# ojcharles/WeightedLD

Measured on AMD Instinct MI355X. Metric: LD site-pairs/sec at N=2000 seq × L=20000 var sites; 1/2/4/8 GPU; %HBM roofline, higher is better.
Workload: dtype fp6 (e2m3) weights x fp4 (e2m1) codes on block-scaled MFMA, screen (f32 sums, exact on the rounded weights; rigorous f32 r2 bound over every pair); candidate tiles (0 of 49144): f32 sums in lib.rs's order on f32 MFMA, f32 epilogue

## Files before the change

weightedld_amd/csrc/pair_mfma.hip:

```cpp
#include <algorithm>
#include <type_traits>
#include <vector>

#include "fp6_pack.hpp"
#include "pair_common.hpp"


namespace wld {

typedef int v4i __attribute__((ext_vector_type(4)));
typedef int v16i __attribute__((ext_vector_type(16)));

bool mfma_supported() { return true; }

namespace {
constexpr int kGroup = 8;
constexpr int kStageCodes = 4096;
constexpr int kDigStage = 128;
constexpr int kMaxPlanes = 4;
constexpr uint32_t kPlanes012 = 0 | (1 << 2) | (2 << 4);
constexpr int kDigGroup = 1024;
template <int NPL>
struct GroupShape {
    static constexpr int kStages = NPL == 1 ? 4 : kGroup;
// ... 821 lines not shown
    }
}
template <bool kShared>
__device__ __forceinline__ void f6c_rebuild(v4f (&acc)[4][2][2], const float2 *sA, const float2 *sB, uint32_t wq,
                                            uint32_t lane, float W6, float wv) {
    float col[4], mb[4];
#pragma unroll
    for (int n = 0; n < 4; ++n) {
        const float2 b = sB[(lane & 15) + 16 * n];
        col[n] = f6c_col_term(b.x, b.y);
        mb[n] = b.y;
    }
#pragma unroll
    for (int e = 0; e < 4; ++e) {
        const float2 a = sA[16 * wq + 4 * (lane >> 4) + e];
        f6c_rebuild_row<kShared>(acc, e, f6c_row_term(W6, a.x), 2.0f * a.y, col, mb, wv);
    }
}
struct F6Site {
    const F6RowRec *row;
    const F6ColRec *col;
    const F6MinRec *rmin, *cmin;
};
template <bool kShared, bool kCounts>
__device__ __forceinline__ void f6c_rebuild_rec(v4f (&acc)[4][2][2], const F6Site &st, uint32_t wq, uint32_t lane,
                                                float wv) {
    float col[4], mb[4];
#pragma unroll
    for (int n = 0; n < 4; ++n) {
        const F6tCol &b = st.col[(lane & 15) + 16 * n].b;
        col[n] = kCounts ? b.col * wv : b.col;
        mb[n] = kCounts ? b.mb * wv : b.mb;
    }
#pragma unroll
    for (int e = 0; e < 4; ++e) {
        const F6tRow &a = st.row[16 * wq + 4 * (lane >> 4) + e].a;
        f6c_rebuild_row<kShared>(acc, e, kCounts ? a.row * wv : a.row, kCounts ? a.ma2 * wv : a.ma2, col, mb, wv);
    }
}
template <bool kShared, bool kCounts>
__device__ __forceinline__ bool f6t_any_doubt(const v4f (&acc)[4][2][2], const F6Epi &ep, const F6Site &st, float wv) {
    F6tCol cb[4];
#pragma unroll
    for (int n = 0; n < 4; ++n) cb[n] = st.col[(ep.lane & 15) + 16 * n].b;
    auto terms = [&](const F6tRow &ra, int n, int e, float &mlo) {
        float p = acc[n][0][1][e], s = acc[n][1][0][e], t = acc[n][1][1][e];
        if constexpr (kCounts)
            p *= 0.5f;
        else if constexpr (kShared)
            p *= 0.5f * wv, s *= wv, t *= wv;
        return r2_screen_terms_f6t(p, s, t, ra, cb[n], ep.thr_c, ep.E, mlo);
    };
    if (ep.okA == ~0ull && ep.okB == ~0ull && ep.ta != ep.tb) {
        int worst = -1;
        float mlo_all = INFINITY;
#pragma unroll
        for (int e = 0; e < 4; ++e) {
            const F6tRow ra = st.row[16 * ep.wq + 4 * (ep.lane >> 4) + e].a;
#pragma unroll
            for (int n = 0; n < 4; ++n) {
                float mlo;
                worst = max(worst, __float_as_int(terms(ra, n, e, mlo)));
                mlo_all = fminf(mlo_all, mlo);
            }
        }
        return worst > 0 || !(mlo_all >= ep.mloc);
    }
    bool doubt = false;
#pragma unroll
    for (int e = 0; e < 4; ++e) {
        const F6tRow ra = st.row[16 * ep.wq + 4 * (ep.lane >> 4) + e].a;
#pragma unroll
        for (int n = 0; n < 4; ++n) {
            float mlo;
            const float t1 = terms(ra, n, e, mlo);
            if (ep.valid_pair(4 * n + e) && (t1 > 0.0f || !(mlo >= ep.mloc))) doubt = true;
        }
    }
    return doubt;
}
struct F6qCol {
    float mb, col, cW;
};
template <bool kShared, bool kCounts>
__device__ __forceinline__ bool f6t_quick_skip(const v4f (&acc)[4][2][2], const F6Epi &ep, const F6Site &st,
                                               const F6qCol (&cb)[4], const F6qColMin &cm, float wv) {
    const uint32_t grp = 4 * ep.wq + (ep.lane >> 4);
    F6qAcc q;
#pragma unroll
    for (int e = 0; e < 4; ++e) {
        const F6tRow &ra = st.row[4 * grp + e].a;
        const float ma2 = ra.ma2, row = ra.row;
#pragma unroll
        for (int n = 0; n < 4; ++n) {
            float p = acc[n][0][1][e], s = acc[n][1][0][e], t = acc[n][1][1][e];
            if constexpr (kShared && !kCounts) p *= 0.5f * wv, s *= wv, t *= wv;
            f6q_pair1<kCounts>(p, s, t, ma2, row, cb[n].mb, cb[n].col, cb[n].cW, q);
            __builtin_amdgcn_sched_barrier(0);
        }
    }
    f6q_pmax<kCounts>(q);
    const F6MinRec r = st.rmin[grp];
    float mlo;
    const float t1 = f6q_lane_terms(q, F6qRowMin{r.x, r.y, r.z}, cm, ep.thr_c, ep.E, mlo);
    return __ballot(!f6q_skip(t1, mlo, ep.mloc)) == 0;
}
template <bool kShared, bool kQuick, bool kCounts>
__device__ __forceinline__ bool f6t_wave_doubt(v4f (&acc)[2][4][2][2], const F6Epi &ep0, const F6Epi &ep1,
                                               const F6Site &st, float wv, uint32_t *full) {
    if constexpr (kQuick) {
        bool full0 = true, full1 = true;
        if (ep0.ta != ep0.tb) {
            F6qCol cb[4];
#pragma unroll
            for (int n = 0; n < 4; ++n) {
                const F6ColRec &b = st.col[(ep0.lane & 15) + 16 * n];
                cb[n] = F6qCol{b.b.mb, b.b.col, b.cW};
            }
            const F6MinRec c = st.cmin[ep0.lane & 15];
            const F6qColMin cm{c.x, c.y, c.z};
            full0 = !f6t_quick_skip<kShared, kCounts>(acc[0], ep0, st, cb, cm, wv);
            full1 = !f6t_quick_skip<kShared, kCounts>(acc[1], ep1, st, cb, cm, wv);
            if ((full0 || full1) && ep0.lane == 0) atomicAdd(full, (uint32_t)full0 + (uint32_t)full1);
        }
        uint32_t lane = ep0.lane;
        asm volatile("" : "+v"(lane), "+s"(wv)::"memory");
#pragma unroll
        for (int j = 0; j < 2; ++j)
#pragma unroll
            for (int n = 0; n < 4; ++n) asm volatile("" : "+v"(acc[j][n][1][1]));
        F6Epi e0 = ep0, e1 = ep1;
        e0.lane = e1.lane = lane;
        return (full0 && f6t_any_doubt<kShared, kCounts>(acc[0], e0, st, wv)) ||
               (full1 && f6t_any_doubt<kShared, kCounts>(acc[1], e1, st, wv));
    }
    return f6t_any_doubt<kShared, kCounts>(acc[0], ep0, st, wv) || f6t_any_doubt<kShared, kCounts>(acc[1], ep1, st, wv);
}
}

template <int kFmt>
__global__ __launch_bounds__(256, 4) void pair_fp6_screen_kernel(const uint8_t *__restrict__ a6,
                                                                  const uint8_t *__restrict__ b6,
                                                                  const float2 *__restrict__ marg, float W6,
                                                                  const uint64_t *__restrict__ ok_bits,
                                                                  const uint32_t *__restrict__ tiles, uint32_t n_tiles,
                                                                  uint32_t NK, uint32_t L, uint32_t n_chunk_rows,
                                                                  float thr, OrderArgs o, ScreenArgs sc, float wv) {
    using F = F6Fmt<kFmt>;
    constexpr int kF6AStage = F::kAStage, kF6ABytes = F::kABytes, kF6Stage = F::kStage;
    __shared__ __attribute__((aligned(16))) uint8_t smem[2 * kF6Stage];
    __shared__ float2 sMarg[2 * kTile];
    __shared__ unsigned long long sMask;
    __shared__ uint32_t sBail;
    if (!sc.probe && blockIdx.x == 0 && threadIdx.x == 0) *sc.cand_work = 0u;
    const uint32_t tid = threadIdx.x, lane = tid & 63, wave = __builtin_amdgcn_readfirstlane(tid >> 6);
    const uint32_t lds = lds_addr(smem), lane16 = lane * 16;
    const uint32_t ei = sc.probe ? blockIdx.x * sc.probe_stride + blockIdx.x % sc.probe_stride : blockIdx.x;
    const uint32_t tile = ei < n_tiles ? tiles[ei] : kNoTile;
    if (tile == kNoTile) return;
    const uint32_t ta = tile >> 16, tb = tile & 0xFFFFu;
    const uint8_t *sA = a6 + (size_t)ta * NK * kF6AStage, *sB = b6 + (size_t)tb * NK * kF6BStage;
    auto issue = [&](uint32_t kb, uint32_t buf) {
        const uint32_t gb = lds + buf * kF6Stage;
        const uint8_t *a = sA + (size_t)kb * kF6AStage, *b = sB + (size_t)kb * kF6BStage;
#pragma unroll
        for (uint32_t p = wave; p < kF6Stage / 1024; p += 4)
            glds16_s(p < kF6AStage / 1024 ? a + p * 1024 : b + (p - kF6AStage / 1024) * kF6BBytes, lane16, gb + p * 1024);
    };
    issue(0, 0);
    if (tid < 2 * kTile) sMarg[tid] = marg[(tid < kTile ? ta : tb) * kTile + (tid & (kTile - 1))];
    if (tid == 0) {
        uint32_t v = 0;
        if (sc.bail) {
            const unsigned cc = __hip_atomic_load(sc.cand_count, __ATOMIC_RELAXED, __HIP_MEMORY_SCOPE_AGENT);
            v = cc > sc.bail ? ((cc & kAbandonBit) ? 2u : 1u) : 0u;
        }
        sBail = v;
    }
    asm volatile("s_waitcnt lgkmcnt(0)" ::: "memory");
    const uint64_t okA = ok_bits[ta], okB = ok_bits[tb];
    v4f acc[4][2][2];
#pragma unroll
    for (int n = 0; n < 4; ++n)
#pragma unroll
        for (int x = 0; x < 2; ++x)
#pragma unroll
            for (int y = 0; y < 2; ++y) acc[n][x][y] = v4f{0.0f, 0.0f, 0.0f, 0.0f};
    uint32_t buf = 0;
    for (uint32_t kb = 0; kb < NK; ++kb) {
        asm volatile("s_waitcnt vmcnt(0)" ::: "memory");
        __builtin_amdgcn_s_barrier();
        asm volatile("" ::: "memory");
        if (kb == 0 && sBail) {
            if (tid == 0 && sBail == 1) {
                atomicOr(sc.cand_count, kAbandonBit);
                atomicOr(sc.cand_buckets, kAbandonBit);
            }
            asm volatile("s_waitcnt vmcnt(0)" ::: "memory");
            return;
        }
        if (kb + 1 < NK) issue(kb + 1, buf ^ 1);
        const uint8_t *g = smem + buf * kF6Stage;
        v8i ai, am;
        f6_ld_rows<kFmt>(g + wave * kF6ABytes, lane, ai, am);
#pragma unroll
        for (int n = 0; n < 4; ++n)
            f6_block_mfma<F::kCbsz>(acc[n], ai, am, f6_ldb(g + kF6AStage + n * kF6BBytes, lane));
        asm volatile("s_waitcnt lgkmcnt(0)" ::: "memory");
        buf ^= 1;
    }
    f6c_rebuild<F::kShared>(acc, sMarg, sMarg + kTile, wave, lane, W6, wv);
    const F6Epi ep{ta, tb, wave, lane, okA, okB, 2.0f * sc.Rf, thr * (1.0f - 0x1p-7f), sc.E, sc.mloc};
    const bool cand = ep.any(acc);
    if (sc.probe) {
        const bool any = __syncthreads_or(cand);
        if (tid == 0) {
            if (any) atomicAdd(sc.probe, 1u);
            atomicAdd(sc.probe + 1, 1u);
        }
        return;
    }
    if (tid == 0) sMask = 0ull;
    if (__syncthreads_or(cand)) {
        const unsigned mk = ep.blocks(acc);
        if (mk) atomicOr(&sMask, (unsigned long long)mk);
        __syncthreads();
        screen_verdict((uint32_t)sMask, ta, tb, tid, n_chunk_rows, o, sc);
    } else {
        screen_verdict(0u, ta, tb, tid, n_chunk_rows, o, sc);
    }
}

constexpr uint32_t kF6Single = 0x8000u;

#ifdef WLD_EXP_CLOCK
constexpr uint32_t kF6ClockSlots = 8192;
__device__ unsigned long long gF6Clock[2 * kF6ClockSlots];
extern "C" int wld_debug_f6_clock(unsigned long long *out) {
    return (int)hipMemcpyFromSymbol(out, HIP_SYMBOL(gF6Clock), sizeof(gF6Clock));
}
#endif
struct F6Recs {
    const F6ColRec *col;
    const F6RowRec *row;
    const F6MinRec *rmin, *cmin;
    float inv;
};
constexpr int kF6SiteCol = 0, kF6SiteRow = 2 * kTile * sizeof(F6ColRec), kF6SiteRmin = kF6SiteRow + kTile * sizeof(F6RowRec),
              kF6SiteCmin = kF6SiteRmin + kTile / 4 * sizeof(F6MinRec),
              kF6SiteBytes = kF6SiteCmin + 2 * 16 * sizeof(F6MinRec);
static_assert(sizeof(F6ColRec) == 32 && sizeof(F6RowRec) == 24 && sizeof(F6MinRec) == 16 && kF6SiteBytes == 6400 &&
                  kF6SiteRow % 16 == 0 && kF6SiteRmin % 16 == 0,
              "the entry's records are staged as 400 16-byte pieces");
__device__ __forceinline__ F6Site f6_site_of(const uint8_t *site, uint32_t half) {
    return F6Site{reinterpret_cast<const F6RowRec *>(site + kF6SiteRow),
                  reinterpret_cast<const F6ColRec *>(site + kF6SiteCol) + kTile * half,
                  reinterpret_cast<const F6MinRec *>(site + kF6SiteRmin),
                  reinterpret_cast<const F6MinRec *>(site + kF6SiteCmin) + 16 * half};
}
template <int kFmt, bool kThree = false, bool kQuick = false, bool kCounts = false>
__global__ __launch_bounds__(256, 3) void pair_fp6_screen2w_kernel(
    const uint8_t *__restrict__ a6, const uint8_t *__restrict__ b6, const float2 *__restrict__ marg, float W6,
    const uint64_t *__restrict__ ok_bits,
    const uint32_t *__restrict__ pairs, uint32_t n_pairs, uint32_t NK, uint32_t L, uint32_t n_chunk_rows, float thr,
    OrderArgs o, ScreenArgs sc, float wv, F6Recs rec) {
    using F = F6Fmt<kFmt>;
    constexpr int kF6AStage = F::kAStage, kF6ABytes = F::kABytes, kF6PStage = F::kPStage;
    static_assert(!kCounts || (kThree && F::kShared), "count units: the shared image's three-sum tests");
    __shared__ __attribute__((aligned(16))) uint8_t smem[2 * kF6PStage];
    __shared__ __attribute__((aligned(kThree ? 16 : 8))) uint8_t sSite[kThree ? kF6SiteBytes : 3 * kTile * sizeof(float2)];
    const float2 *const sMarg = reinterpret_cast<const float2 *>(sSite);
    __shared__ unsigned long long sMask[2];
    __shared__ uint32_t sBail, sCand[2];
    __shared__ uint32_t sDoubt[2];
    __shared__ uint32_t sQuickFull;
    static_assert(kThree || !kQuick, "the quick test stands in front of the three-sum test");
    if (!sc.probe && blockIdx.x == 0 && threadIdx.x == 0) *sc.cand_work = 0u;
    const uint32_t tid = threadIdx.x, lane = tid & 63, wave = __builtin_amdgcn_readfirstlane(tid >> 6);
    const uint32_t half = wave >> 1, rp = wave & 1, ltid = tid & 127;
    const uint32_t lds = lds_addr(smem), lane16 = lane * 16;
    const uint32_t ei = sc.probe ? blockIdx.x * sc.probe_stride + blockIdx.x % sc.probe_stride : blockIdx.x;
    const uint32_t entry = ei < n_pairs ? pairs[ei] : kNoTile;
    if (entry == kNoTile) return;
    constexpr int kAPieces = kFmt == kF6A6 ? 3 : kFmt == kF6A4 ? 2 : 1;
    static_assert(kF6AStage == kAPieces * 4096 && kF6BStage == 4096, "five (fp4 A: four, shared: three) pieces per wave and stage");
    struct Src {
        const uint8_t *pA, *pB0, *pB1;
    };
    auto src_of = [&](uint32_t e) {
        const uint32_t ta_ = e >> 16, tb0_ = e & 0x7FFFu;
        Src r;
        r.pA = a6 + (size_t)ta_ * NK * kF6AStage + wave * 1024;
        r.pB0 = b6 + (size_t)tb0_ * NK * kF6BStage + wave * 1024;
        r.pB1 = (e & kF6Single) ? r.pB0 : r.pB0 + (size_t)NK * kF6BStage;
        return r;
    };
    auto issue = [&](const Src &sr, uint32_t kb, uint32_t buf) {
        const uint32_t gb = lds + buf * kF6PStage + wave * 1024;
        const uint8_t *a = sr.pA + (size_t)kb * kF6AStage;
        const size_t bo = (size_t)kb * kF6BStage;
        glds16_s(a, lane16, gb);
        if (kAPieces > 1) glds16_s(a + 4096, lane16, gb + 4096);
        if (kAPieces > 2) glds16_s(a + 8192, lane16, gb + 8192);
        glds16_s(sr.pB0 + bo, lane16, gb + kF6AStage);
        glds16_s(sr.pB1 + bo, lane16, gb + kF6AStage + kF6BStage);
    };
    const Src cur = src_of(entry);
    issue(cur, 0, 0);
    uint32_t buf = 0;
    {
        const uint32_t ta = entry >> 16, tb0 = entry & 0x7FFFu;
        const bool single = (entry & kF6Single) != 0, idle = single && half;
        const uint32_t tb = tb0 + (idle ? 0u : half);
        if constexpr (kThree) {
            const uint32_t tb1 = tb0 + (single ? 0u : 1u);
            uint4 *const dst = reinterpret_cast<uint4 *>(sSite);
            dst[tid] = reinterpret_cast<const uint4 *>(rec.col + (tid < 128 ? tb0 : tb1) * kTile)[tid & 127];
            if (tid < 96)
                dst[kF6SiteRow / 16 + tid] = reinterpret_cast<const uint4 *>(rec.row + ta * kTile)[tid];
            else if (tid < 112)
                dst[kF6SiteRmin / 16 + (tid - 96)] = reinterpret_cast<const uint4 *>(rec.rmin + ta * (kTile / 4))[tid - 96];
            else if (tid < 144)
                dst[kF6SiteCmin / 16 + (tid - 112)] =
                    reinterpret_cast<const uint4 *>(rec.cmin + (tid < 128 ? tb0 : tb1) * 16)[tid & 15];
        } else if (tid < 3 * kTile) {
            const uint32_t t = tid < kTile ? ta : tb0 + ((tid >= 2 * kTile && !single) ? 1u : 0u);
            reinterpret_cast<float2 *>(sSite)[tid] = marg[t * kTile + (tid & (kTile - 1))];
        }
        if (tid == 0) {
            uint32_t v = 0;
            if (sc.bail) {
                const unsigned cc = __hip_atomic_load(sc.cand_count, __ATOMIC_RELAXED, __HIP_MEMORY_SCOPE_AGENT);
                v = cc > sc.bail ? ((cc & kAbandonBit) ? 2u : 1u) : 0u;
            }
            sBail = v;
        }
        if constexpr (kThree)
            if (tid < 2) sDoubt[tid] = 0u;
        if constexpr (kQuick)
            if (tid == 2) sQuickFull = 0u;
        asm volatile("s_waitcnt lgkmcnt(0)" ::: "memory");
        const uint64_t okA = ok_bits[ta], okB = ok_bits[tb];
        v4f acc[2][4][2][2];
        const uint32_t boff = kF6AStage + (idle ? 0u : half) * kF6BStage;
        const uint32_t aoff = 2 * rp * kF6ABytes;
        auto stage = [&](uint32_t kb, auto first) -> bool {
            constexpr bool kFirst = decltype(first)::value;
            asm volatile("s_waitcnt vmcnt(0)" ::: "memory");
            __builtin_amdgcn_s_barrier();
            asm volatile("" ::: "memory");
            if (kFirst) {
                if (sBail) {
                    if (tid == 0 && sBail == 1) {
                        atomicOr(sc.cand_count, kAbandonBit);
                        atomicOr(sc.cand_buckets, kAbandonBit);
                    }
                    asm volatile("s_waitcnt vmcnt(0)" ::: "memory");
                    return false;
                }
                if (tid < 2) sCand[tid] = 0u, sMask[tid] = 0ull;
            }
            if (kb + 1 < NK) issue(cur, kb + 1, buf ^ 1);
            const uint8_t *g = smem + buf * kF6PStage;
            v8i ai0, am0, ai1, am1;
            f6_ld_rows<kFmt>(g + aoff, lane, ai0, am0);
            f6_ld_rows<kFmt>(g + aoff + kF6ABytes, lane, ai1, am1);
            const v4f kZero = {0.0f, 0.0f, 0.0f, 0.0f};
            v8i bs[2] = {f6_ldb(g + boff, lane), f6_ldb(g + boff + kF6BBytes, lane)};
#pragma unroll
            for (int n = 0; n < 4; ++n) {
                v8i &b = bs[n & 1];
                constexpr int kMinor = 0x22222222;
                if constexpr (!kThree) acc[0][n][0][0] = f6_mfma<F::kCbsz>(ai0, b, kFirst ? kZero : acc[0][n][0][0]);
                acc[0][n][1][0] = f6_mfma<F::kCbsz>(am0, b, kFirst ? kZero : acc[0][n][1][0]);
                if constexpr (!kThree) acc[1][n][0][0] = f6_mfma<F::kCbsz>(ai1, b, kFirst ? kZero : acc[1][n][0][0]);
                acc[1][n][1][0] = f6_mfma<F::kCbsz>(am1, b, kFirst ? kZero : acc[1][n][1][0]);
                __builtin_amdgcn_sched_barrier(0);
                b = v8i{b[0] & kMinor, b[1] & kMinor, b[2] & kMinor, b[3] & kMinor, 0, 0, 0, 0};
                acc[0][n][0][1] = f6_mfma<F::kCbsz>(ai0, b, kFirst ? kZero : acc[0][n][0][1]);
                acc[0][n][1][1] = f6_mfma<F::kCbsz>(am0, b, kFirst ? kZero : acc[0][n][1][1]);
                acc[1][n][0][1] = f6_mfma<F::kCbsz>(ai1, b, kFirst ? kZero : acc[1][n][0][1]);
                acc[1][n][1][1] = f6_mfma<F::kCbsz>(am1, b, kFirst ? kZero : acc[1][n][1][1]);
                __builtin_amdgcn_sched_barrier(0);
                if (n + 2 < 4) b = f6_ldb(g + boff + (n + 2) * kF6BBytes, lane);
                __builtin_amdgcn_sched_barrier(0);
            }
            asm volatile("s_waitcnt lgkmcnt(0)" ::: "memory");
            buf ^= 1;
            return true;
        };
#ifdef WLD_EXP_CLOCK
        const unsigned long long ck0 = clock64(), rt0 = wall_clock64();
#endif
        if (!stage(0, std::true_type{})) return;
        for (uint32_t kb = 1; kb < NK; ++kb) stage(kb, std::false_type{});
#ifdef WLD_EXP_CLOCK
        if (tid == 0) {
            gF6Clock[2 * (blockIdx.x % kF6ClockSlots)] = clock64() - ck0;
            gF6Clock[2 * (blockIdx.x % kF6ClockSlots) + 1] = wall_clock64() - rt0;
        }
#endif
        const F6Epi ep0{ta, tb, 2 * rp, lane, okA, okB, 2.0f * sc.Rf, thr * (1.0f - 0x1p-7f), sc.E, sc.mloc};
        const F6Epi ep1{ta, tb, 2 * rp + 1, lane, okA, okB, 2.0f * sc.Rf, thr * (1.0f - 0x1p-7f), sc.E, sc.mloc};
        if constexpr (kThree) {
            const F6Site st = f6_site_of(sSite, half);
            F6Epi t0 = ep0, t1 = ep1;
            t0.E = t1.E = kCounts ? sc.E * rec.inv * rec.inv : sc.E;
            t0.mloc = t1.mloc = kCounts ? sc.mloc * rec.inv : sc.mloc;
            const bool doubt =
                !idle && f6t_wave_doubt<F::kShared, kQuick, kCounts>(acc, t0, t1, st, wv, &sQuickFull);
            if (doubt) sDoubt[half] = 1u;
            __syncthreads();
            if constexpr (kQuick) {
                unsigned *const cnt = sc.probe ? sc.probe + 3 : sc.rechecked ? sc.rechecked + 1 : nullptr;
                if (tid == 0 && cnt && sQuickFull) atomicAdd(cnt, sQuickFull);
            }
#ifdef WLD_EXP_ZERO_IMG
            const bool again = (sDoubt[0] | sDoubt[1]) == 0x5EEDu;
#else
            const bool again = (sDoubt[0] | sDoubt[1]) != 0;
#endif
            if (!again) {
                if (sc.probe) {
                    if (ltid == 0 && !idle) atomicAdd(sc.probe + 1, 1u);
                } else if (!idle) {
                    screen_verdict(0u, ta, tb, ltid, n_chunk_rows, o, sc);
                }
                return;
            }
            if (unsigned *const cnt = sc.probe ? sc.probe + 2 : sc.rechecked; tid == 0 && cnt) atomicAdd(cnt, 1u);
#pragma unroll
            for (int n = 0; n < 4; ++n) acc[0][n][0][0] = acc[1][n][0][0] = v4f{0.0f, 0.0f, 0.0f, 0.0f};
            issue(cur, 0, buf);
            for (uint32_t kb = 0; kb < NK; ++kb) {
                asm volatile("s_waitcnt vmcnt(0)" ::: "memory");
                __builtin_amdgcn_s_barrier();
                asm volatile("" ::: "memory");
                if (kb + 1 < NK) issue(cur, kb + 1, buf ^ 1);
                const uint8_t *g = smem + buf * kF6PStage;
                v8i ai0, ai1;
                if constexpr (F::kShared) {
                    v8i am0, am1;
                    f6_ld_rows<kFmt>(g + aoff, lane, ai0, am0);
                    f6_ld_rows<kFmt>(g + aoff + kF6ABytes, lane, ai1, am1);
                } else {
                    ai0 = f6_lda<kFmt>(g + aoff, lane);
                    ai1 = f6_lda<kFmt>(g + aoff + kF6ABytes, lane);
                }
#pragma unroll
                for (int n = 0; n < 4; ++n) {
                    const v8i b = f6_ldb(g + boff + n * kF6BBytes, lane);
                    acc[0][n][0][0] = f6_mfma<F::kCbsz>(ai0, b, acc[0][n][0][0]);
                    acc[1][n][0][0] = f6_mfma<F::kCbsz>(ai1, b, acc[1][n][0][0]);
                }
                asm volatile("s_waitcnt lgkmcnt(0)" ::: "memory");
                buf ^= 1;
            }
        }
        if (!idle) {
            if constexpr (kThree) {
                const F6Site st = f6_site_of(sSite, half);
                f6c_rebuild_rec<F::kShared, kCounts>(acc[0], st, 2 * rp, lane, wv);
                f6c_rebuild_rec<F::kShared, kCounts>(acc[1], st, 2 * rp + 1, lane, wv);
            } else {
                f6c_rebuild<F::kShared>(acc[0], sMarg, sMarg + kTile * (1 + half), 2 * rp, lane, W6, wv);
                f6c_rebuild<F::kShared>(acc[1], sMarg, sMarg + kTile * (1 + half), 2 * rp + 1, lane, W6, wv);
            }
        }
        const bool cand = !idle && (ep0.any(acc[0]) || ep1.any(acc[1]));
        if (cand) sCand[half] = 1u;
        __syncthreads();
#ifdef WLD_EXP_ZERO_IMG
        const bool mine = sCand[half] == 0x5EEDu;
#else
        const bool mine = sCand[half] != 0;
#endif
        if (sc.probe) {
            if (ltid == 0 && !idle) {
                if (mine) atomicAdd(sc.probe, 1u);
                atomicAdd(sc.probe + 1, 1u);
            }
            return;
        }
        if (mine && !idle) {
            const unsigned mk = ep0.blocks(acc[0]) | ep1.blocks(acc[1]);
            if (mk) atomicOr(&sMask[half], (unsigned long long)mk);
        }
        __syncthreads();
        if (!idle) screen_verdict(mine ? (uint32_t)sMask[half] : 0u, ta, tb, ltid, n_chunk_rows, o, sc);
    }
}

constexpr int kI8ABytes = 2048;
constexpr int kI8AStage = 4 * kI8ABytes;
constexpr int kI8BStage = 4 * 1024;
constexpr int kI8PStage = kI8AStage + 2 * kI8BStage;
size_t i8_a_bytes(size_t LP, size_t NP) { return LP / 64 * (NP / 64) * kI8AStage; }
size_t i8_b_bytes(size_t LP, size_t NP) { return LP / 64 * (NP / 64) * kI8BStage; }

__global__ __launch_bounds__(256) void i8img_kernel(const uint8_t *__restrict__ codes, const int8_t *__restrict__ digit,
                                                     uint32_t LP, uint32_t NP, uint8_t *__restrict__ a8,
                                                     uint8_t *__restrict__ b8) {
    const uint32_t NK = NP / 64;
    const size_t idx = (size_t)blockIdx.x * 256 + threadIdx.x;
    if (idx >= (size_t)LP / 16 * NK * 64) return;
    const uint32_t lane = idx & 63, blk = (idx >> 6) & 3;
    const size_t tk = idx >> 8, tile = tk / NK;
    const uint32_t kb = (uint32_t)(tk % NK);
    const uint32_t k0 = 64 * kb + 16 * (lane >> 4);
    const uint4 c4 = *reinterpret_cast<const uint4 *>(codes + (tile * 64 + blk * 16 + (lane & 15)) * (size_t)NP + k0);
    const uint4 d4 = *reinterpret_cast<const uint4 *>(digit + k0);
    const uint32_t c[4] = {c4.x, c4.y, c4.z, c4.w}, d[4] = {d4.x, d4.y, d4.z, d4.w};
    uint32_t ai[4], am[4], b[4];
#pragma unroll
    for (int q = 0; q < 4; ++q) {
        uint32_t vi = 0, vm = 0, vb = 0;
#pragma unroll
        for (int j = 0; j < 4; ++j) {
            const uint32_t cc = (c[q] >> (8 * j)) & 0xFFu, dd = (d[q] >> (8 * j)) & 0xFFu;
            vi |= ((cc & kCodeIn) ? dd : 0u) << (8 * j);
            vm |= ((cc & kCodeMaj) ? dd : 0u) << (8 * j);
            vb |= ((cc & kCodeIn) ? ((cc & kCodeMaj) ? 2u : 1u) : 0u) << (8 * j);
        }
        ai[q] = vi, am[q] = vm, b[q] = vb;
    }
    uint8_t *pa = a8 + tk * kI8AStage + blk * kI8ABytes;
    *reinterpret_cast<uint4 *>(pa + 16 * lane) = make_uint4(ai[0], ai[1], ai[2], ai[3]);
    *reinterpret_cast<uint4 *>(pa + 1024 + 16 * lane) = make_uint4(am[0], am[1], am[2], am[3]);
    *reinterpret_cast<uint4 *>(b8 + tk * kI8BStage + blk * 1024 + 16 * lane) = make_uint4(b[0], b[1], b[2], b[3]);
}

void launch_i8img(const uint8_t *codes, const int8_t *digit, size_t LP, size_t NP, uint8_t *a8, uint8_t *b8,
                  hipStream_t s) {
    const size_t n = LP / 16 * (NP / 64) * 64;
    hipLaunchKernelGGL(i8img_kernel, dim3((unsigned)((n + 255) / 256)), dim3(256), 0, s, codes, digit, (uint32_t)LP,
                       (uint32_t)NP, a8, b8);
}

__global__ __launch_bounds__(256, 3) void pair_i8_screen2w_kernel(
    const uint8_t *__restrict__ a8, const uint8_t *__restrict__ b8, const uint64_t *__restrict__ ok_bits,
    const uint32_t *__restrict__ pairs, uint32_t n_pairs, uint32_t NK, uint32_t L, uint32_t n_chunk_rows, float thr,
    OrderArgs o, ScreenArgs sc) {
    __shared__ __attribute__((aligned(16))) uint8_t smem[2 * kI8PStage];
    __shared__ unsigned long long sMask[2];
    __shared__ uint32_t sCand[2];
    if (blockIdx.x == 0 && threadIdx.x == 0) *sc.cand_work = 0u;
    const uint32_t tid = threadIdx.x, lane = tid & 63, wave = __builtin_amdgcn_readfirstlane(tid >> 6);
    const uint32_t half = wave >> 1, rp = wave & 1, ltid = tid & 127;
    const uint32_t lds = lds_addr(smem), lane16 = lane * 16;
    const uint32_t entry = blockIdx.x < n_pairs ? pairs[blockIdx.x] : kNoTile;
    if (entry == kNoTile) return;
    const uint32_t ta = entry >> 16, tb0 = entry & 0x7FFFu;
    const bool single = (entry & kF6Single) != 0, idle = single && half;
    const uint32_t tb = tb0 + (idle ? 0u : half);
    static_assert(kI8AStage == 2 * 4096 && kI8BStage == 4096, "four pieces per wave and stage");
    const uint8_t *pA = a8 + (size_t)ta * NK * kI8AStage + wave * 1024;
    const uint8_t *pB0 = b8 + (size_t)tb0 * NK * kI8BStage + wave * 1024;
    const uint8_t *pB1 = single ? pB0 : pB0 + (size_t)NK * kI8BStage;
    auto issue = [&](uint32_t kb, uint32_t buf) {
        const uint32_t gb = lds + buf * kI8PStage + wave * 1024;
        const uint8_t *a = pA + (size_t)kb * kI8AStage;
        const size_t bo = (size_t)kb * kI8BStage;
        glds16_s(a, lane16, gb);
// ... 171 lines not shown
    hipLaunchKernelGGL(frag_kernel, dim3((unsigned)((chunks + 255) / 256)), dim3(256), 0, s, codes, (uint32_t)LP,
                       (uint32_t)NP, frag);
}

int mfma_weight_stats(const int8_t *wplanes, size_t LP, size_t NP, hipStream_t s, MfmaWeightStats *out) {
    struct {
        unsigned mask, pad;
        unsigned long long resid[3];
        unsigned long long dsum[kMaxPlanes];
    } h{};
    if (hipMemcpyAsync(&h, wplanes + planemask_offset(LP, NP), sizeof(h), hipMemcpyDeviceToHost, s) != hipSuccess ||
        hipStreamSynchronize(s) != hipSuccess)
        return -1;
    out->plane_mask = h.mask & 15;
    out->nonneg = !(h.mask & 0x100);
    for (int t = 0; t < 3; ++t) out->resid[t] = h.resid[t];
    for (int p = 0; p < kMaxPlanes; ++p) out->dsum[p] = h.dsum[p];
    return 0;
}

namespace {
template <int MODE, int NPL, bool LOOP = false>
void launch_lds(const MfmaLaunch &m, const uint64_t *ok_bits, const uint32_t *tiles, uint32_t n_tiles,
                const unsigned *tile_count, uint32_t grid, uint32_t plane_idx, const OrderArgs &o, const DenseArgs &dn,
                const ScreenArgs &sc, hipStream_t s) {
    hipLaunchKernelGGL((pair_mfma_kernel<MODE, NPL, LOOP>), dim3(grid), dim3(64 * GroupShape<NPL>::kWaves), 0, s, m.frag, m.frag_b, m.wplanes,
                       ok_bits, tiles, n_tiles, tile_count, m.L, m.NP, m.n_chunk_rows, m.thr, m.shift, plane_idx, o,
                       dn, sc);
}

template <int MODE, bool LOOP = false>
void launch_lds_planes(uint32_t n_planes, const MfmaLaunch &m, const uint64_t *ok_bits, const uint32_t *tiles,
                       uint32_t n_tiles, const unsigned *tile_count, uint32_t grid, uint32_t plane_idx,
                       const OrderArgs &o, const DenseArgs &dn, const ScreenArgs &sc, hipStream_t s) {
    if (n_planes == 4)
        launch_lds<MODE, 4, LOOP>(m, ok_bits, tiles, n_tiles, tile_count, grid, plane_idx, o, dn, sc, s);
    else if (n_planes == 3)
        launch_lds<MODE, 3, LOOP>(m, ok_bits, tiles, n_tiles, tile_count, grid, plane_idx, o, dn, sc, s);
    else if (n_planes == 2 || LOOP)
        launch_lds<MODE, 2, LOOP>(m, ok_bits, tiles, n_tiles, tile_count, grid, plane_idx, o, dn, sc, s);
    else
        launch_lds<MODE, 1, false>(m, ok_bits, tiles, n_tiles, tile_count, grid, plane_idx, o, dn, sc, s);
}
void launch_candidates(const MfmaLaunch &m, uint32_t n, uint32_t idx, const uint64_t *ok_bits, const OrderArgs &o,
                       const DenseArgs &dn, const ScreenArgs &sc, hipStream_t s) {
    if (m.test_guard && sc.cand_buckets && m.cand_list && sc.cand_bits && sc.cand_cap) {
        const size_t cap = sc.cand_cap, last = 16 * (size_t)m.n_tiles / cap - 1;
        (void)hipMemsetD32Async(reinterpret_cast<hipDeviceptr_t>(m.cand_list + last * cap), 0, cap, s);
        (void)hipMemsetD32Async(reinterpret_cast<hipDeviceptr_t>(sc.cand_bits + last * cap), 0, cap, s);
        (void)hipMemsetD32Async(reinterpret_cast<hipDeviceptr_t>(sc.cand_buckets + last), (int)(cap + 1), 1, s);
        if (m.cand_count)
            (void)hipMemsetD32Async(reinterpret_cast<hipDeviceptr_t>(m.cand_count), (int)(16 * m.n_tiles + 2), 1, s);
    }
    if (m.ref_valu) {
        ValuLaunch v = *m.ref_valu;
        v.tiles = m.cand_list;
        v.n_tiles = m.n_tiles;
        v.tile_count = m.cand_count;
        v.tile_bits = sc.cand_bits;
        v.tile_work = sc.cand_work;
        v.tile_buckets = sc.cand_buckets;
        v.bucket_cap = sc.cand_cap;
        v.rb_items = sc.rb_items != 0;
        v.scan = sc.scan;
        launch_pair_valu(v, o, nullptr, s);
        return;
    }
    const uint32_t grid = std::min<uint32_t>(m.n_tiles, kCandidateGrid);
    launch_lds_planes<kModePrefilter, true>(n, m, ok_bits, m.cand_list, 0, m.cand_count, grid, idx, o, dn, sc, s);
}
}

namespace {
void fp6_screen_args(const MfmaLaunch &m, ScreenArgs &sc) {
    sc.R = fp6_screen_R(*m.fp6);
    sc.Rf = (float)sc.R;
    sc.f32 = 2;
    screen_consts(m.fp6->Tg, 2.0f * sc.Rf, sc.E, sc.mloc);
}
template <int kFmt>
void launch_fp6_screen_fmt(const MfmaLaunch &m, const uint64_t *ok_bits, const OrderArgs &o, const ScreenArgs &sc,
                           uint32_t stride, hipStream_t s) {
    const bool counts = kFmt == kF6Shared && m.fp6->counts;
    const F6Recs rec = fp6_recs_of(m.fp6->rec, m.LP, counts ? 1.0f / m.fp6->wv : 1.0f);
    auto pairs = [&](auto kernel) {
        hipLaunchKernelGGL(kernel, dim3((m.f6_n_pairs + stride - 1) / stride), dim3(256), 0, s, m.fp6->a6, m.fp6->b6,
                           reinterpret_cast<const float2 *>(m.fp6->marg), m.fp6->W6, ok_bits, m.f6_pairs, m.f6_n_pairs,
                           m.fp6->NK, m.L, m.n_chunk_rows, m.thr, o, sc, m.fp6->wv, rec);
    };
    if (m.f6_pairs && m.fp6_three && m.fp6_quick) {
        if constexpr (kFmt == kF6Shared) {
            if (counts) return pairs(pair_fp6_screen2w_kernel<kFmt, true, true, true>);
        }
        pairs(pair_fp6_screen2w_kernel<kFmt, true, true>);
    } else if (m.f6_pairs && m.fp6_three) {
        if constexpr (kFmt == kF6Shared) {
            if (counts) return pairs(pair_fp6_screen2w_kernel<kFmt, true, false, true>);
        }
        pairs(pair_fp6_screen2w_kernel<kFmt, true>);
    } else if (m.f6_pairs) {
        pairs(pair_fp6_screen2w_kernel<kFmt>);
    } else {
        hipLaunchKernelGGL(pair_fp6_screen_kernel<kFmt>, dim3((m.n_tiles + stride - 1) / stride), dim3(256), 0, s,
                           m.fp6->a6, m.fp6->b6, reinterpret_cast<const float2 *>(m.fp6->marg), m.fp6->W6, ok_bits,
                           m.tiles, m.n_tiles, m.fp6->NK, m.L, m.n_chunk_rows, m.thr,
                           o, sc, m.fp6->wv);
    }
}
void launch_fp6_screen(const MfmaLaunch &m, const uint64_t *ok_bits, const OrderArgs &o, const ScreenArgs &sc,
                       uint32_t stride, hipStream_t s) {
    if (m.fp6->shared)
        launch_fp6_screen_fmt<kF6Shared>(m, ok_bits, o, sc, stride, s);
    else if (m.fp6->a4)
        launch_fp6_screen_fmt<kF6A4>(m, ok_bits, o, sc, stride, s);
    else
        launch_fp6_screen_fmt<kF6A6>(m, ok_bits, o, sc, stride, s);
}
}

void launch_fp6_probe(const MfmaLaunch &m, unsigned *probe, uint32_t stride, hipStream_t s) {
    const uint64_t *ok_bits = reinterpret_cast<const uint64_t *>(m.wplanes + okbits_offset(m.NP));
    ScreenArgs sc{};
    sc.nonneg = m.nonneg;
    fp6_screen_args(m, sc);
    sc.probe = probe;
    sc.probe_stride = std::max<uint32_t>(stride, 1);
    (void)hipMemsetAsync(probe, 0, 4 * sizeof(unsigned), s);
    launch_fp6_screen(m, ok_bits, OrderArgs{}, sc, sc.probe_stride, s);
}

void launch_pair_mfma(const MfmaLaunch &m, const OrderArgs &o, const DenseArgs *dense, hipStream_t s,
                      hipEvent_t screen_done) {
    using screen_policy::Route;
    const DenseArgs dn = dense ? *dense : DenseArgs{nullptr, nullptr, nullptr, nullptr};
    const uint64_t *ok_bits = reinterpret_cast<const uint64_t *>(m.wplanes + okbits_offset(m.NP));
    ScreenArgs sc{0.0,         0.0f,         0.0f,      0.0f,        0, m.nonneg, m.cand_list, m.cand_count,
                  m.cand_list + 16 * (size_t)m.n_tiles, m.cand_work, m.cand_buckets, m.n_tiles, 0, ScanArgs{}};
    if (!m.frag) {
        const dim3 g(m.n_tiles), b(256);
        if (dense)
            hipLaunchKernelGGL((pair_mfma_rows_kernel<kModeDense>), g, b, 0, s, m.codes, m.wplanes, ok_bits, m.tiles,
                               m.L, m.NP, m.n_chunk_rows, m.thr, m.shift, o, dn, sc);
        else if (m.bound_test)
            hipLaunchKernelGGL((pair_mfma_rows_kernel<kModePrefilter>), g, b, 0, s, m.codes, m.wplanes, ok_bits,
                               m.tiles, m.L, m.NP, m.n_chunk_rows, m.thr, m.shift, o, dn, sc);
        else
            hipLaunchKernelGGL((pair_mfma_rows_kernel<kModeAll>), g, b, 0, s, m.codes, m.wplanes, ok_bits, m.tiles,
                               m.L, m.NP, m.n_chunk_rows, m.thr, m.shift, o, dn, sc);
        return;
    }
    unsigned mask = m.plane_mask & 15;
    if (!mask) mask = 15;
    uint32_t idx = 0, n = 0, top = 0;
    for (uint32_t p = 0; p < kMaxPlanes; ++p)
        if (mask >> p & 1) idx |= p << (2 * n++), top = p;
    if (n == 3 && idx != kPlanes012) n = 4;
    if (n == 4) idx = 0 | (1 << 2) | (2 << 4) | (3 << 6);
    if (dense) {
        launch_lds_planes<kModeDense>(n, m, ok_bits, m.tiles, m.n_tiles, nullptr, m.n_tiles, idx, o, dn, sc, s);
        return;
    }
    if (!m.bound_test) {
        launch_lds_planes<kModeAll>(n, m, ok_bits, m.tiles, m.n_tiles, nullptr, m.n_tiles, idx, o, dn, sc, s);
        return;
    }
    const auto begin_screen = [&] {
        sc.scan = m.scan;
        if (m.ref_valu && !m.ref_valu->safe) {
            sc.rb_items = 1;
            sc.cand_cap = 4 * m.n_tiles;
        }
// ... 72 lines not shown
```

Baseline: 519.9 billion.

## Overlap screen kernel prologue: async record staging, early bail load, prefetched row records

The fp6 screen kernel's prologue is reorganized. The kernel-argument fields it needs first are gathered into a compact head struct and pinned to scalar registers. The per-tile site records are now staged into LDS with direct global-to-LDS loads, issued after the next k-stage load (or at once when NK==1), instead of synchronous uint4 copies followed by an lgkmcnt wait. The bail counter is read before the first stage and published at that stage's barrier, and the quick-skip epilogue software-prefetches the next row record inside its loop. The goal is to hide global load latency and launch overhead in short blocks, at the cost of more complex ordering and waitcnt assumptions. Clock instrumentation is extended as well.

```diff
diff --git a/weightedld_amd/csrc/pair_mfma.hip b/weightedld_amd/csrc/pair_mfma.hip
--- a/weightedld_amd/csrc/pair_mfma.hip
+++ b/weightedld_amd/csrc/pair_mfma.hip
@@ -927,15 +927,27 @@
 struct F6qCol {
     float mb, col, cW;
 };
-template <bool kShared, bool kCounts>
+struct F6qRow {
+    float ma2, row;
+};
+__device__ __forceinline__ F6qRow f6q_row_of(const F6Site &st, uint32_t site) {
+    const F6tRow &ra = st.row[site].a;
+    return F6qRow{ra.ma2, ra.row};
+}
+template <bool kShared, bool kCounts, bool kNext>
 __device__ __forceinline__ bool f6t_quick_skip(const v4f (&acc)[4][2][2], const F6Epi &ep, const F6Site &st,
-                                               const F6qCol (&cb)[4], const F6qColMin &cm, float wv) {
+                                               const F6qCol (&cb)[4], const F6qColMin &cm, float wv, F6qRow &nx) {
     const uint32_t grp = 4 * ep.wq + (ep.lane >> 4);
+    const F6MinRec r = st.rmin[grp];
     F6qAcc q;
 #pragma unroll
     for (int e = 0; e < 4; ++e) {
-        const F6tRow &ra = st.row[4 * grp + e].a;
-        const float ma2 = ra.ma2, row = ra.row;
+        const float ma2 = nx.ma2, row = nx.row;
+        if (e < 3)
+            nx = f6q_row_of(st, 4 * grp + e + 1);
+        else if (kNext)
+            nx = f6q_row_of(st, 4 * (grp + 4));
+        __builtin_amdgcn_sched_barrier(0);
 #pragma unroll
         for (int n = 0; n < 4; ++n) {
             float p = acc[n][0][1][e], s = acc[n][1][0][e], t = acc[n][1][1][e];
@@ -945,7 +957,6 @@
         }
     }
     f6q_pmax<kCounts>(q);
-    const F6MinRec r = st.rmin[grp];
     float mlo;
     const float t1 = f6q_lane_terms(q, F6qRowMin{r.x, r.y, r.z}, cm, ep.thr_c, ep.E, mlo);
     return __ballot(!f6q_skip(t1, mlo, ep.mloc)) == 0;
@@ -964,8 +975,9 @@
             }
             const F6MinRec c = st.cmin[ep0.lane & 15];
             const F6qColMin cm{c.x, c.y, c.z};
-            full0 = !f6t_quick_skip<kShared, kCounts>(acc[0], ep0, st, cb, cm, wv);
-            full1 = !f6t_quick_skip<kShared, kCounts>(acc[1], ep1, st, cb, cm, wv);
+            F6qRow nx = f6q_row_of(st, 4 * (4 * ep0.wq + (ep0.lane >> 4)));
+            full0 = !f6t_quick_skip<kShared, kCounts, true>(acc[0], ep0, st, cb, cm, wv, nx);
+            full1 = !f6t_quick_skip<kShared, kCounts, false>(acc[1], ep1, st, cb, cm, wv, nx);
             if ((full0 || full1) && ep0.lane == 0) atomicAdd(full, (uint32_t)full0 + (uint32_t)full1);
         }
         uint32_t lane = ep0.lane;
@@ -1079,11 +1091,26 @@
 constexpr uint32_t kF6Single = 0x8000u;
 
 #ifdef WLD_EXP_CLOCK
-constexpr uint32_t kF6ClockSlots = 8192;
-__device__ unsigned long long gF6Clock[2 * kF6ClockSlots];
+constexpr uint32_t kF6ClockSlots = 8192, kF6ClockWords = 10;
+__device__ unsigned long long gF6Clock[kF6ClockWords * kF6ClockSlots];
 extern "C" int wld_debug_f6_clock(unsigned long long *out) {
     return (int)hipMemcpyFromSymbol(out, HIP_SYMBOL(gF6Clock), sizeof(gF6Clock));
 }
+#define F6_CLOCK_BEGIN unsigned long long ck[8] = {}; const unsigned long long rt0 = wall_clock64(); ck[0] = clock64()
+#define F6_STAMP(i) ck[i] = clock64()
+#define F6_CLOCK_END                                                                         \
+    do {                                                                                     \
+        ck[7] = clock64();                                                                   \
+        if (threadIdx.x == 0) {                                                              \
+            unsigned long long *const g = gF6Clock + kF6ClockWords * (blockIdx.x % kF6ClockSlots); \
+            for (int i = 0; i < 8; ++i) g[i] = ck[i];                                        \
+            g[8] = rt0, g[9] = wall_clock64();                                               \
+        }                                                                                    \
+    } while (0)
+#else
+#define F6_CLOCK_BEGIN (void)0
+#define F6_STAMP(i) (void)0
+#define F6_CLOCK_END (void)0
 #endif
 struct F6Recs {
     const F6ColRec *col;
@@ -1103,12 +1130,23 @@
                   reinterpret_cast<const F6MinRec *>(site + kF6SiteRmin),
                   reinterpret_cast<const F6MinRec *>(site + kF6SiteCmin) + 16 * half};
 }
+struct F6Head {
+    const uint32_t *pairs;
+    const uint8_t *a6, *b6;
+    const uint8_t *rec;
+    unsigned *probe;
+    const unsigned *cand_count;
+    const uint64_t *ok_bits;
+    uint32_t n_pairs, NK, probe_stride, bail;
+    uint32_t LP;
+    float inv;
+};
 template <int kFmt, bool kThree = false, bool kQuick = false, bool kCounts = false>
 __global__ __launch_bounds__(256, 3) void pair_fp6_screen2w_kernel(
-    const uint8_t *__restrict__ a6, const uint8_t *__restrict__ b6, const float2 *__restrict__ marg, float W6,
-    const uint64_t *__restrict__ ok_bits,
-    const uint32_t *__restrict__ pairs, uint32_t n_pairs, uint32_t NK, uint32_t L, uint32_t n_chunk_rows, float thr,
-    OrderArgs o, ScreenArgs sc, float wv, F6Recs rec) {
+    F6Head hd, const float2 *__restrict__ marg, float W6, uint32_t L, uint32_t n_chunk_rows, float thr, OrderArgs o,
+    ScreenArgs sc, float wv) {
+    const uint8_t *const a6 = hd.a6, *const b6 = hd.b6;
+    const uint32_t NK = hd.NK;
     using F = F6Fmt<kFmt>;
     constexpr int kF6AStage = F::kAStage, kF6ABytes = F::kABytes, kF6PStage = F::kPStage;
     static_assert(!kCounts || (kThree && F::kShared), "count units: the shared image's three-sum tests");
@@ -1120,13 +1158,20 @@
     __shared__ uint32_t sDoubt[2];
     __shared__ uint32_t sQuickFull;
     static_assert(kThree || !kQuick, "the quick test stands in front of the three-sum test");
-    if (!sc.probe && blockIdx.x == 0 && threadIdx.x == 0) *sc.cand_work = 0u;
+    F6_CLOCK_BEGIN;
+    asm volatile("" ::"s"(hd.pairs), "s"(hd.a6), "s"(hd.b6), "s"(hd.rec), "s"(hd.probe), "s"(hd.cand_count),
+                 "s"(hd.ok_bits), "s"(hd.n_pairs), "s"(hd.NK), "s"(hd.probe_stride), "s"(hd.bail), "s"(hd.LP));
     const uint32_t tid = threadIdx.x, lane = tid & 63, wave = __builtin_amdgcn_readfirstlane(tid >> 6);
     const uint32_t half = wave >> 1, rp = wave & 1, ltid = tid & 127;
     const uint32_t lds = lds_addr(smem), lane16 = lane * 16;
-    const uint32_t ei = sc.probe ? blockIdx.x * sc.probe_stride + blockIdx.x % sc.probe_stride : blockIdx.x;
-    const uint32_t entry = ei < n_pairs ? pairs[ei] : kNoTile;
-    if (entry == kNoTile) return;
+    const uint32_t ei = hd.probe ? blockIdx.x * hd.probe_stride + blockIdx.x % hd.probe_stride : blockIdx.x;
+    const uint32_t entry = ei < hd.n_pairs ? hd.pairs[ei] : kNoTile;
+    if (entry == kNoTile) {
+        if (!hd.probe && blockIdx.x == 0 && threadIdx.x == 0) *sc.cand_work = 0u;
+        return;
+    }
+    unsigned bail_cc = 0;
+    if (hd.bail && tid == 0) bail_cc = __hip_atomic_load(hd.cand_count, __ATOMIC_RELAXED, __HIP_MEMORY_SCOPE_AGENT);
     constexpr int kAPieces = kFmt == kF6A6 ? 3 : kFmt == kF6A4 ? 2 : 1;
     static_assert(kF6AStage == kAPieces * 4096 && kF6BStage == 4096, "five (fp4 A: four, shared: three) pieces per wave and stage");
     struct Src {
@@ -1152,48 +1197,63 @@
     };
     const Src cur = src_of(entry);
     issue(cur, 0, 0);
+    F6_STAMP(1);
     uint32_t buf = 0;
     {
         const uint32_t ta = entry >> 16, tb0 = entry & 0x7FFFu;
         const bool single = (entry & kF6Single) != 0, idle = single && half;
         const uint32_t tb = tb0 + (idle ? 0u : half);
-        if constexpr (kThree) {
-            const uint32_t tb1 = tb0 + (single ? 0u : 1u);
-            uint4 *const dst = reinterpret_cast<uint4 *>(sSite);
-            dst[tid] = reinterpret_cast<const uint4 *>(rec.col + (tid < 128 ? tb0 : tb1) * kTile)[tid & 127];
-            if (tid < 96)
-                dst[kF6SiteRow / 16 + tid] = reinterpret_cast<const uint4 *>(rec.row + ta * kTile)[tid];
-            else if (tid < 112)
-                dst[kF6SiteRmin / 16 + (tid - 96)] = reinterpret_cast<const uint4 *>(rec.rmin + ta * (kTile / 4))[tid - 96];
-            else if (tid < 144)
-                dst[kF6SiteCmin / 16 + (tid - 112)] =
-                    reinterpret_cast<const uint4 *>(rec.cmin + (tid < 128 ? tb0 : tb1) * 16)[tid & 15];
-        } else if (tid < 3 * kTile) {
-            const uint32_t t = tid < kTile ? ta : tb0 + ((tid >= 2 * kTile && !single) ? 1u : 0u);
-            reinterpret_cast<float2 *>(sSite)[tid] = marg[t * kTile + (tid & (kTile - 1))];
-        }
-        if (tid == 0) {
-            uint32_t v = 0;
-            if (sc.bail) {
-                const unsigned cc = __hip_atomic_load(sc.cand_count, __ATOMIC_RELAXED, __HIP_MEMORY_SCOPE_AGENT);
-                v = cc > sc.bail ? ((cc & kAbandonBit) ? 2u : 1u) : 0u;
-            }
-            sBail = v;
+        auto issue_recs = [&]() {
+            if constexpr (kThree) {
+                static_assert(kF6SiteCol == 0 && kF6SiteRow == 256 * 16 && kF6SiteRmin == (256 + 96) * 16 &&
+                                  kF6SiteCmin == (256 + 112) * 16 && kF6SiteBytes == (256 + 144) * 16,
+                              "the piece map below");
+                const uint32_t tb1 = tb0 + (single ? 0u : 1u);
+                const uint32_t sl = lds_addr(sSite) + wave * 1024;
+                const size_t row = (size_t)hd.LP * sizeof(F6ColRec), rmin = row + (size_t)hd.LP * sizeof(F6RowRec),
+                             cmin = rmin + (size_t)hd.LP / 4 * sizeof(F6MinRec);
+                glds16_s(hd.rec + ((size_t)(half ? tb1 : tb0) * (kTile * sizeof(F6ColRec)) + rp * 1024), lane16, sl);
+                if (wave == 0) {
+                    glds16_s(hd.rec + row + (size_t)ta * (kTile * sizeof(F6RowRec)), lane16, sl + kF6SiteRow);
+                } else if (wave == 1) {
+                    const uint32_t r1 = (uint32_t)row + ta * (uint32_t)(kTile * sizeof(F6RowRec)) + 1024,
+                                   m1 = (uint32_t)rmin + ta * (uint32_t)(kTile / 4 * sizeof(F6MinRec)) - 32 * 16,
+                                   c1 = (uint32_t)cmin + tb0 * (uint32_t)(16 * sizeof(F6MinRec)) - 48 * 16;
+                    glds16_s(hd.rec, (lane < 32 ? r1 : lane < 48 ? m1 : c1) + lane16, sl + kF6SiteRow);
+                } else if (wave == 2) {
+                    if (lane < 16)
+                        glds16_s(hd.rec + cmin + (size_t)tb1 * (16 * sizeof(F6MinRec)), lane16, sl + kF6SiteRow);
+                }
+            }
+        };
+        if (NK == 1) issue_recs();
+        if (!hd.probe && blockIdx.x == 0 && tid == 0) *sc.cand_work = 0u;
+        if constexpr (!kThree) {
+            if (tid < 3 * kTile) {
+                const uint32_t t = tid < kTile ? ta : tb0 + ((tid >= 2 * kTile && !single) ? 1u : 0u);
+                reinterpret_cast<float2 *>(sSite)[tid] = marg[t * kTile + (tid & (kTile - 1))];
+            }
         }
         if constexpr (kThree)
             if (tid < 2) sDoubt[tid] = 0u;
         if constexpr (kQuick)
             if (tid == 2) sQuickFull = 0u;
-        asm volatile("s_waitcnt lgkmcnt(0)" ::: "memory");
-        const uint64_t okA = ok_bits[ta], okB = ok_bits[tb];
+        const uint64_t okA = hd.ok_bits[ta], okB = hd.ok_bits[tb];
+        asm volatile("" ::"s"(thr), "s"(wv), "s"(sc.Rf), "s"(sc.E), "s"(sc.mloc), "s"(n_chunk_rows));
         v4f acc[2][4][2][2];
         const uint32_t boff = kF6AStage + (idle ? 0u : half) * kF6BStage;
         const uint32_t aoff = 2 * rp * kF6ABytes;
         auto stage = [&](uint32_t kb, auto first) -> bool {
             constexpr bool kFirst = decltype(first)::value;
             asm volatile("s_waitcnt vmcnt(0)" ::: "memory");
+            if (kFirst) {
+                if (tid == 0) sBail = bail_cc > hd.bail ? ((bail_cc & kAbandonBit) ? 2u : 1u) : 0u;
+                asm volatile("s_waitcnt lgkmcnt(0)" ::: "memory");
+            }
+            if (kFirst) F6_STAMP(2);
             __builtin_amdgcn_s_barrier();
             asm volatile("" ::: "memory");
+            if (kFirst) F6_STAMP(3);
             if (kFirst) {
                 if (sBail) {
                     if (tid == 0 && sBail == 1) {
@@ -1205,7 +1265,10 @@
                 }
                 if (tid < 2) sCand[tid] = 0u, sMask[tid] = 0ull;
             }
-            if (kb + 1 < NK) issue(cur, kb + 1, buf ^ 1);
+            if (kb + 1 < NK) {
+                issue(cur, kb + 1, buf ^ 1);
+                if (kFirst) issue_recs();
+            }
             const uint8_t *g = smem + buf * kF6PStage;
             v8i ai0, am0, ai1, am1;
             f6_ld_rows<kFmt>(g + aoff, lane, ai0, am0);
@@ -1234,30 +1297,24 @@
             buf ^= 1;
             return true;
         };
-#ifdef WLD_EXP_CLOCK
-        const unsigned long long ck0 = clock64(), rt0 = wall_clock64();
-#endif
         if (!stage(0, std::true_type{})) return;
         for (uint32_t kb = 1; kb < NK; ++kb) stage(kb, std::false_type{});
-#ifdef WLD_EXP_CLOCK
-        if (tid == 0) {
-            gF6Clock[2 * (blockIdx.x % kF6ClockSlots)] = clock64() - ck0;
-            gF6Clock[2 * (blockIdx.x % kF6ClockSlots) + 1] = wall_clock64() - rt0;
-        }
-#endif
+        F6_STAMP(4);
         const F6Epi ep0{ta, tb, 2 * rp, lane, okA, okB, 2.0f * sc.Rf, thr * (1.0f - 0x1p-7f), sc.E, sc.mloc};
         const F6Epi ep1{ta, tb, 2 * rp + 1, lane, okA, okB, 2.0f * sc.Rf, thr * (1.0f - 0x1p-7f), sc.E, sc.mloc};
         if constexpr (kThree) {
             const F6Site st = f6_site_of(sSite, half);
             F6Epi t0 = ep0, t1 = ep1;
-            t0.E = t1.E = kCounts ? sc.E * rec.inv * rec.inv : sc.E;
-            t0.mloc = t1.mloc = kCounts ? sc.mloc * rec.inv : sc.mloc;
+            t0.E = t1.E = kCounts ? sc.E * hd.inv * hd.inv : sc.E;
+            t0.mloc = t1.mloc = kCounts ? sc.mloc * hd.inv : sc.mloc;
             const bool doubt =
                 !idle && f6t_wave_doubt<F::kShared, kQuick, kCounts>(acc, t0, t1, st, wv, &sQuickFull);
+            F6_STAMP(5);
             if (doubt) sDoubt[half] = 1u;
             __syncthreads();
+            F6_STAMP(6);
             if constexpr (kQuick) {
-                unsigned *const cnt = sc.probe ? sc.probe + 3 : sc.rechecked ? sc.rechecked + 1 : nullptr;
+                unsigned *const cnt = hd.probe ? hd.probe + 3 : sc.rechecked ? sc.rechecked + 1 : nullptr;
                 if (tid == 0 && cnt && sQuickFull) atomicAdd(cnt, sQuickFull);
             }
 #ifdef WLD_EXP_ZERO_IMG
@@ -1266,14 +1323,15 @@
             const bool again = (sDoubt[0] | sDoubt[1]) != 0;
 #endif
             if (!again) {
-                if (sc.probe) {
-                    if (ltid == 0 && !idle) atomicAdd(sc.probe + 1, 1u);
+                if (hd.probe) {
+                    if (ltid == 0 && !idle) atomicAdd(hd.probe + 1, 1u);
                 } else if (!idle) {
                     screen_verdict(0u, ta, tb, ltid, n_chunk_rows, o, sc);
                 }
+                F6_CLOCK_END;
                 return;
             }
-            if (unsigned *const cnt = sc.probe ? sc.probe + 2 : sc.rechecked; tid == 0 && cnt) atomicAdd(cnt, 1u);
+            if (unsigned *const cnt = hd.probe ? hd.probe + 2 : sc.rechecked; tid == 0 && cnt) atomicAdd(cnt, 1u);
 #pragma unroll
             for (int n = 0; n < 4; ++n) acc[0][n][0][0] = acc[1][n][0][0] = v4f{0.0f, 0.0f, 0.0f, 0.0f};
             issue(cur, 0, buf);
@@ -1320,10 +1378,10 @@
 #else
         const bool mine = sCand[half] != 0;
 #endif
-        if (sc.probe) {
+        if (hd.probe) {
             if (ltid == 0 && !idle) {
-                if (mine) atomicAdd(sc.probe, 1u);
-                atomicAdd(sc.probe + 1, 1u);
+                if (mine) atomicAdd(hd.probe, 1u);
+                atomicAdd(hd.probe + 1, 1u);
             }
             return;
         }
@@ -1661,11 +1719,12 @@
 void launch_fp6_screen_fmt(const MfmaLaunch &m, const uint64_t *ok_bits, const OrderArgs &o, const ScreenArgs &sc,
                            uint32_t stride, hipStream_t s) {
     const bool counts = kFmt == kF6Shared && m.fp6->counts;
-    const F6Recs rec = fp6_recs_of(m.fp6->rec, m.LP, counts ? 1.0f / m.fp6->wv : 1.0f);
+    const F6Head hd{m.f6_pairs, m.fp6->a6, m.fp6->b6, static_cast<const uint8_t *>(m.fp6->rec), sc.probe, sc.cand_count,
+                    ok_bits, m.f6_n_pairs, m.fp6->NK, sc.probe_stride, sc.bail, (uint32_t)m.LP, counts ? 1.0f / m.fp6->wv : 1.0f};
     auto pairs = [&](auto kernel) {
-        hipLaunchKernelGGL(kernel, dim3((m.f6_n_pairs + stride - 1) / stride), dim3(256), 0, s, m.fp6->a6, m.fp6->b6,
-                           reinterpret_cast<const float2 *>(m.fp6->marg), m.fp6->W6, ok_bits, m.f6_pairs, m.f6_n_pairs,
-                           m.fp6->NK, m.L, m.n_chunk_rows, m.thr, o, sc, m.fp6->wv, rec);
+        hipLaunchKernelGGL(kernel, dim3((m.f6_n_pairs + stride - 1) / stride), dim3(256), 0, s, hd,
+                           reinterpret_cast<const float2 *>(m.fp6->marg), m.fp6->W6, m.L, m.n_chunk_rows, m.thr, o, sc,
+                           m.fp6->wv);
     };
     if (m.f6_pairs && m.fp6_three && m.fp6_quick) {
         if constexpr (kFmt == kF6Shared) {
```

Result: no change. 519.4 billion (median of 2 runs) (-0.1%).
